# instadeepai/FrameDiPT

Hardware: AMD Instinct MI355X
Metric: residue*diffusion-steps/sec (higher is better)
Workload: dtype fp16

## Files before the change

### framedipt_amd/csrc/edge_transition4.hip

```cpp
#include <type_traits>

#include "common.hpp"
#include "kernels.hpp"

#define E4_CZ 128
#define E4_H 384
#define E4_WAVES 8
#define E4_THREADS (64 * E4_WAVES)
#define E4_BUF 32768
#define E4_WBI (2048 + 64)
#define E4_L1_FR (12 * 8)
#define E4_L2_FR (12 * 24)
#define E4_LF_FR (24 * 4)
#define E4_DZ_FR0 496
#define E4_STREAM_FR 512
#define E4_STREAM_BYTES (E4_STREAM_FR * 1024)
static_assert(E4_L1_FR + E4_L2_FR + E4_LF_FR == 480, "480 weight fragments, then one unused chunk and the down_z chunk");
#define E4X_LF_FR (24 * 8)
#define E4X_DZ_FR0 624
#define E4X_STREAM_FR 640
#define E4X_STREAM_BYTES (E4X_STREAM_FR * 1024)
static_assert(E4_L1_FR + E4_L2_FR + E4X_LF_FR == 576 && E4X_DZ_FR0 + 16 == E4X_STREAM_FR, "fp16x stream: 36 weight chunks, down_z in the last");
#define E4_ZOFF (2 * E4_BUF)
#define E4_VOFF (E4_ZOFF + E4_WAVES * 8192)
// ... 326 lines not shown
        float* bo = a.bias_out + fd_bias_frag_off((long)b * a.H + 4 * half, nt, ii, jj);
        const long hstride = (long)nt * nt * 1024;
        const f32x4 bbv = e4_ldsf4(bbo + 16 * half);
#pragma unroll
        for (int r = 0; r < 4; ++r)
          if (4 * half + r < a.H) bo[r * hstride] = X.accb[r] + bbv[r];
      }
    }
    if constexpr (PZ) {
      const int NJ4 = a.N >> 2;
#pragma unroll
      for (int g = 0; g < 4; ++g) {
        const int row = 8 * E.t.rt + 2 * g + half;
        const u32x2 ow = {fd_cvt_pk(X.accd[4 * g], X.accd[4 * g + 1]), fd_cvt_pk(X.accd[4 * g + 2], X.accd[4 * g + 3])};
        if (E.t.valid && row < M)
          *(u32x2*)(a.pz_out + (((long)row * NJ4 + E.t.jt) * 32 + p) * 4) = ow;
      }
    }
  }
}

#define E4_DR 4
#define E4_CHUNK 16384
#define E4_NSLOT 4
#define E4_NCHUNK 32
#define E4_CFR (E4_CHUNK / 1024)
#define E4_DZ_LDS 49152u
#define E4_DPC (E4_CHUNK / (E4_THREADS * 16))
__device__ __forceinline__ void e4_vm_wait(int n) {
  __builtin_amdgcn_sched_barrier(0);
#define E4_VMC(k) case k: __builtin_amdgcn_s_waitcnt(0x0F70 | ((k) & 15) | (((k) >> 4) << 14)); break;
  switch (n) {
    E4_VMC(1) E4_VMC(2) E4_VMC(3) E4_VMC(4) E4_VMC(5) E4_VMC(6) E4_VMC(7) E4_VMC(8) E4_VMC(9) E4_VMC(10) E4_VMC(11) E4_VMC(12)
    E4_VMC(13) E4_VMC(14) E4_VMC(15) E4_VMC(16) E4_VMC(17) E4_VMC(18) E4_VMC(19) E4_VMC(20)
    default: __builtin_amdgcn_s_waitcnt(0x0F70); break;
  }
#undef E4_VMC
  __builtin_amdgcn_sched_barrier(0);
}
#define E4_PT_Z 24
#define E4_PT_FL 26
__device__ __forceinline__ constexpr int e4_vm_younger(int c) {
  return (E4_NSLOT - 3) * E4_DPC + (c > E4_PT_Z && c <= E4_PT_Z + E4_NSLOT - 2 ? 8 : (c > E4_PT_FL && c <= E4_PT_FL + E4_NSLOT - 2 ? 4 : (c <= E4_NSLOT - 3 ? 14 : 0)));
}
__device__ __forceinline__ constexpr unsigned e4_ring_off(int f) { return (unsigned)(((f / E4_CFR) % E4_NSLOT) * E4_CHUNK + (f % E4_CFR) * 1024); }
struct E4Flat {
  const char* stream;
  unsigned lds0, pa;
  int tid, wave;
};
template <int NCH = E4_NCHUNK>
__device__ __forceinline__ void e4_point(const E4Flat& F, int c) {
  e4_vm_wait(e4_vm_younger(c));
  __builtin_amdgcn_s_barrier();
  __builtin_amdgcn_sched_barrier(0);
  const int cn = (c + E4_NSLOT - 1) % NCH;
  e4_dma_chunk<E4_CHUNK>(F.stream + (size_t)cn * E4_CHUNK, F.lds0 + (unsigned)(cn % E4_NSLOT) * E4_CHUNK, F.tid, F.wave);
}
#define E4_STEP(f_, B_, acc_)                                                                                   \
  do {                                                                                                          \
    if ((f_) + E4_DR - 1 < NCH * E4_CFR) r[((f_) + E4_DR - 1) % E4_DR] = fd_frag(F.pa + e4_ring_off((f_) + E4_DR - 1)); \
    acc_ = fd_mfma32(r[(f_) % E4_DR], B_, acc_);                                                                  \
    __builtin_amdgcn_sched_barrier(0);                                                                          \
  } while (0)

template <bool PZ, bool STZ = true, bool LO = false>
__global__ __launch_bounds__(E4_THREADS, 8 / E4_WAVES) void edge_transition4_flat_kernel(ET2Args a, int n_tiles, int n_wt) {
  constexpr int NCH = (LO ? E4X_STREAM_FR : E4_STREAM_FR) / E4_CFR;
  constexpr int LFW = LO ? 8 : 4;
  extern __shared__ __attribute__((aligned(16))) char smem[];
  const unsigned lds0 = (unsigned)(unsigned long)(__attribute__((address_space(3))) char*)smem;
  const unsigned vec = lds0 + E4_VOFF;
  const unsigned wbi = lds0 + E4_VOFF + E4_VEC_BYTES;
  const int wave = __builtin_amdgcn_readfirstlane(threadIdx.x >> 6);
  auto lane_id = [] {
    int l = __builtin_amdgcn_mbcnt_hi(~0u, __builtin_amdgcn_mbcnt_lo(~0u, 0u));
    asm volatile("" : "+v"(l));
    return l;
  };
  const int lane0 = lane_id(), tid0 = wave * 64 + lane0;
  const int N = a.N, NJ4 = N >> 2, M = a.B * N;
  const char* stream = (const char*)a.stream;
  int tile = blockIdx.x;
  if (tile >= n_tiles) return;
  E4_CLK_BEGIN;
#ifdef E4_PROF
  unsigned ph[8] = {0, 0, 0, 0, 0, 0, 0, 0}, tlast = (unsigned)__builtin_amdgcn_s_memtime();
  const unsigned long long span0 = __builtin_amdgcn_s_memrealtime();
#endif
  E4Tile tc = e4_tile_of(tile * E4_WAVES + wave, n_wt, N, NJ4);
  e4_request_z(a, tc, lane0, lds0 + E4_ZOFF + wave * 8192, M);
#pragma unroll
  for (int c = 0; c < E4_NSLOT - 1; ++c) e4_dma_chunk<E4_CHUNK>(stream + c * E4_CHUNK, lds0 + c * E4_CHUNK, tid0, wave);
  if (tid0 < (PZ ? 168 : 160)) {
    const float* src = tid0 < 96 ? a.b2 + 4 * tid0 : (tid0 < 128 ? a.gamma + 4 * (tid0 - 96) : (tid0 < 160 ? a.beta + 4 * (tid0 - 128) : a.bdz + 4 * (tid0 - 160)));
    fd_dma16(src, vec + (tid0 & ~63) * 16);
  }
  if (a.wb_img && tid0 < 128) fd_dma16((const char*)a.wb_img + tid0 * 16, wbi + (tid0 & ~63) * 16);
  if (tid0 < 4) *(__attribute__((address_space(3))) unsigned*)(unsigned long)(wbi + 2048 + tid0 * 4) = 0u;
  auto fold_ptr = [&](const E4Tile& t, int lane) {
    const unsigned fold_b1 = (unsigned)((const char*)a.b1_img - (const char*)a.a1_img);
    const unsigned ob = fold_b1 + (unsigned)((t.b0 * NJ4 + t.jt) * 16) * 512u, oa = (unsigned)(t.rt * 16) * 512u;
    return oa + (unsigned)(lane >> 5) * (ob - oa) + (lane & 31) * 16;
  };
  auto fold_ld = [&](unsigned off) { return fd_frag((const char*)a.a1_img + off); };
  unsigned fold_base = fold_ptr(tc, lane0);
  hx8 FA[12];
#pragma unroll
  for (int k = 0; k < 12; ++k) FA[k] = fold_ld(fold_base + k * 512);
  auto mask_of = [&](const E4Tile& t, int lane) {
    int row = 8 * t.rt + ((lane & 31) >> 2);
    if (row > M - 1) row = M - 1;
    return a.res_mask[row] * a.res_mask[(row / N) * N + 4 * t.jt + (lane & 3)];
  };
  if (tid0 < 8) *(__attribute__((address_space(3))) float*)(unsigned long)(lds0 + E4_BOFF + tid0 * 4) = (a.wb_img && tid0 < a.H) ? a.bb[tid0] : 0.f;
  float em_req = mask_of(tc, lane0);
  E4Epi E;
  E4EpiTmp X;
#define E4_EPI(k, emr) e4_epi<k, PZ, STZ, emr>(E, X, a, lane_id(), vec, wbi, lds0 + E4_SOFF + wave * 2048, M, lds0 + E4_DZ_LDS)
  fd_dma_wait();
  *(__attribute__((address_space(3))) float*)(unsigned long)(lds0 + E4_MOFF + tid0 * 4) = em_req;
  __syncthreads();
  E4_STAMP(0);
#pragma unroll 1
  for (;;) {
    const int lane = lane_id(), tid = wave * 64 + lane;
    const int p = lane & 31, half = lane >> 5;
    const unsigned zst = lds0 + E4_ZOFF + wave * 8192;
    const unsigned zrow = zst + p * 256;
    E4Flat F;
    F.stream = stream; F.lds0 = lds0; F.pa = lds0 + lane * 16; F.tid = tid; F.wave = wave;
    hx8 r[E4_DR];
#pragma unroll
    for (int m = 0; m < E4_DR - 1; ++m) r[m] = fd_frag(F.pa + e4_ring_off(m));
    hx8 H1[24], H2[24];
    {
      const hx8 SEL = e4_sel(lane, tc.ns);
      hx8 Zf[8];
#pragma unroll
      for (int s = 0; s < 8; ++s) Zf[s] = fd_frag(zrow + (((2 * s) ^ (half ^ (p & 15))) << 4));
      __builtin_amdgcn_sched_barrier(0);
#pragma unroll
      for (int T = 0; T < 12; ++T) {
        f32x16 acc;
#pragma unroll
        for (int q = 0; q < 16; ++q) acc[q] = 0.f;
        acc = fd_mfma32(FA[T], SEL, acc);
#pragma unroll
        for (int s = 0; s < 8; ++s) {
          const int f = 8 * T + s;
          if (f % E4_CFR == E4_CFR / 2) e4_point<NCH>(F, f / E4_CFR);
          E4_STEP(f, Zf[s], acc);
        }
        fd_hand_off(acc, H1[2 * T], H1[2 * T + 1]);
        __builtin_amdgcn_sched_barrier(0);
      }
    }
    E4_STAMP(1);
#pragma unroll
    for (int T = 0; T < 12; ++T) {
      f32x16 acc;
#pragma unroll
      for (int g = 0; g < 4; ++g) {
        const f32x4 bv = e4_ldsf4(vec + 4 * (32 * T + 8 * g + 4 * half));
#pragma unroll
        for (int q = 0; q < 4; ++q) acc[4 * g + q] = bv[q];
      }
#pragma unroll
      for (int s = 0; s < 24; ++s) {
        const int f = E4_L1_FR + 24 * T + s;
        if (f % E4_CFR == E4_CFR / 2) e4_point<NCH>(F, f / E4_CFR);
        E4_STEP(f, H1[s], acc);
      }
      fd_hand_off(acc, H2[2 * T], H2[2 * T + 1]);
      __builtin_amdgcn_sched_barrier(0);
      if (T < 4) {
        const int l3 = lane_id();
        const unsigned zrow3 = lds0 + E4_ZOFF + wave * 8192 + (l3 & 31) * 256 + 8 * (l3 >> 5), zsw = l3 & 15;
#pragma unroll
        for (int u = 0; u < 2; ++u) {
          u32x4 zw;
          const u32x2 z0 = *(e4_lds_w64)(unsigned long)(zrow3 + (((4 * T + 2 * u) ^ zsw) << 4));
          const u32x2 z1 = *(e4_lds_w64)(unsigned long)(zrow3 + (((4 * T + 2 * u + 1) ^ zsw) << 4));
          zw[0] = z0[0]; zw[1] = z0[1]; zw[2] = z1[0]; zw[3] = z1[1];
          H2[2 * T + u] = H2[2 * T + u] + __builtin_bit_cast(hx8, zw);
        }
      }
    }
    E4_STAMP(2);
    const int ntile = tile + gridDim.x;
    const bool has_next = ntile < n_tiles;
    const E4Tile tn = e4_tile_of((has_next ? ntile : tile) * E4_WAVES + wave, n_wt, N, NJ4);
#pragma unroll
    for (int t = 0; t < 4; ++t)
#pragma unroll
      for (int q = 0; q < 16; ++q) E.Y[t][q] = 0.f;
    hx8 FL[4];
#pragma unroll
    for (int s = 0; s < 24; ++s)
#pragma unroll
      for (int u = 0; u < LFW; ++u) {
        const int t = u & 3;
        const int f = E4_L1_FR + E4_L2_FR + LFW * s + u;
        if (f % E4_CFR == E4_CFR / 2) {
          e4_point<NCH>(F, f / E4_CFR);
          if (f / E4_CFR == E4_PT_Z) e4_request_z(a, tn, lane_id(), lds0 + E4_ZOFF + wave * 8192, M);
          if (f / E4_CFR == E4_PT_FL) {
            const unsigned fb = fold_ptr(tc, lane_id());
#pragma unroll
            for (int k = 0; k < 4; ++k) FL[k] = fold_ld(fb + (12 + k) * 512);
          }
        }
        E4_STEP(f, H2[s], E.Y[t]);
      }
    static_assert((E4_L1_FR + E4_L2_FR + 24 * LFW) / E4_CFR == NCH - (LO ? 4 : 2), "stream points behind the final layer");
    if constexpr (LO) {
      e4_point<NCH>(F, NCH - 4);
      e4_point<NCH>(F, NCH - 3);
    }
    e4_point<NCH>(F, NCH - 2);
    e4_point<NCH>(F, NCH - 1);
    {
      const hx8 SEL = e4_sel(lane, tc.ns);
#pragma unroll
      for (int t = 0; t < 4; ++t) E.Y[t] = fd_mfma32(FL[t], SEL, E.Y[t]);
    }
    E4_STAMP(3);
    fold_base = fold_ptr(tn, lane);
#pragma unroll
    for (int k = 0; k < 12; ++k) FA[k] = fold_ld(fold_base + k * 512);
    E.t = tc;
    em_req = mask_of(tn, lane);
    X.moff = lds0 + E4_MOFF + tid * 4;
    X.boff = lds0 + E4_BOFF;
    E4_EPI(0, true); E4_EPI(1, true); E4_EPI(2, true); E4_EPI(3, true); E4_EPI(4, true); E4_EPI(5, true); E4_EPI(6, true);
    E4_STAMP(4);
    if (!has_next) break;
    tile = ntile;
    tc = tn;
    e4_vm_wait(14);
    *(__attribute__((address_space(3))) float*)(unsigned long)(lds0 + E4_MOFF + tid * 4) = em_req;
    E4_STAMP(5);
  }
  fd_dma_wait();
  E4_CLK_END;
#ifdef E4_PROF
  if (tid0 == 0 && blockIdx.x < 256)
    for (int k = 0; k < 8; ++k) e4_prof[blockIdx.x * 8 + k] = ph[k];
  if (tid0 == 0 && blockIdx.x < 1024) {
    e4_span[blockIdx.x * 3] = span0;
    e4_span[blockIdx.x * 3 + 1] = __builtin_amdgcn_s_memrealtime();
    e4_span[blockIdx.x * 3 + 2] = 0;
  }
#endif
}

int fd_edge_transition4_supported(int N) { return N >= 8 && N <= 2048 && N % 4 == 0; }

template <bool LO>
static int e4_launch(const ET2Args& a, hipStream_t st) {
  const int n_wt = ((a.B * a.N + 7) / 8) * (a.N / 4);
  const int n_tiles = cdiv(n_wt, E4_WAVES);
  static FdPerDevice attr_dev;
  const int dev_ = fd_device();
  if (!attr_dev.get(dev_)) {
    if (hipFuncSetAttribute((const void*)edge_transition4_flat_kernel<false, true, LO>, hipFuncAttributeMaxDynamicSharedMemorySize, E4_LDS) != hipSuccess ||
        hipFuncSetAttribute((const void*)edge_transition4_flat_kernel<true, true, LO>, hipFuncAttributeMaxDynamicSharedMemorySize, E4_LDS) != hipSuccess ||
        hipFuncSetAttribute((const void*)edge_transition4_flat_kernel<true, false, LO>, hipFuncAttributeMaxDynamicSharedMemorySize, E4_LDS) != hipSuccess)
      return FDIPT_ELAUNCH;
    attr_dev.set(dev_, 1);
  }
  const int n_cu = fd_cu_count();
  const int cus = a.reserve_cus > 0 && a.reserve_cus < n_cu - 8 ? (n_cu - a.reserve_cus) & ~7 : n_cu;
// ... 26 lines not shown
```

### framedipt_amd/csrc/kernels.hpp

```cpp
#pragma once
#include <hip/hip_runtime.h>
#include <stdint.h>

typedef unsigned short half_t;

struct EdgeTransArgs {
  int B, N;
  const void* z_in;
  void* z_out;
  const float* e;
  const void *w1, *w2, *wf;
  const float *b1, *b2, *bf, *gamma, *beta;
  const float* res_mask;
  float* trace;
  unsigned long long* clock = nullptr;
};

struct EdgeEmbedArgs {
  int B, N, n_rel, rel_off, num_bins;
  const float* pi;
  const float* pj;
  const float* rtab;
  const float* dtab;
  const float* edges;
// ... 69 lines not shown
  unsigned short* kpf = nullptr;
  const float* gamma = nullptr;
  const float* res_mask = nullptr;
};
#define FD_KPF_FRAGS 4

__host__ __device__ __forceinline__ long fd_bias_frag_off(long bh, int nt, int i, int j) {
  return ((((bh * nt + (i >> 5)) * nt + (j >> 5)) * 32 + (i & 31)) * 32) + (j & 31);
}

struct ET2Args {
  int B, N;
  const half_t* z_in;
  half_t* z_out;
  const float* e;
  const half_t* e_h16;
  const float* a1;
  const float* af;
  const void* stream;
  const float *b2, *gamma, *beta, *res_mask;
  float* trace;
  const void* wb_img;
  const float* bb;
  float* bias_out;
  int H;
  const void* a1_img;
  const void* b1_img;
  int reserve_cus = 0;
  unsigned long long* clock = nullptr;
  const void* wdz_img = nullptr;
  const void* wdz_img_lo = nullptr;
  const float* bdz = nullptr;
  half_t* pz_out = nullptr;
};
static inline size_t fd_pz_bytes(int B, int N) { return (size_t)B * N * ((N + 3) / 4) * 256; }
int fd_et3_build_stream(const float* w1, const float* w2, const float* wf, void* stream, hipStream_t st);
size_t fd_et3_stream_bytes();
int fd_edge_transition3(const ET2Args& a, hipStream_t st);
int fd_et3_build_bias_image(const float* wb, int H, float scale, void* img, hipStream_t st);
int fd_edge_transition3_supported(int N);
int fd_et4_build_stream(const float* w1, const float* w2, const float* wf, void* stream, hipStream_t st, int lo = 0);
int fd_et4_set_dz(void* stream, const void* img_hi, const void* img_lo, hipStream_t st, int lo = 0);
size_t fd_et4_stream_bytes(int lo = 0);
int fd_et4_build_bias_image(const float* wb, int H, float scale, void* img, hipStream_t st);
size_t fd_et4_a_image_bytes(int B, int N);
size_t fd_et4_b_image_bytes(int B, int N);
int fd_et4_row_images(const float* rows, int B, int N, void* a_img, void* b_img, hipStream_t st);
int fd_edge_transition4(const ET2Args& a, hipStream_t st, int lo = 0);
int fd_edge_transition4_supported(int N);
int fd_ee2_build_images(const float* w2, const float* w3, void* img, hipStream_t st, int lo = 0);
size_t fd_ee2_image_bytes(int lo = 0);
int fd_edge_embed2(const EdgeEmbedArgs& a, const void* img, hipStream_t st, int lo = 0);

struct ProjArgs {
  int B, N, H, C, K, PT, Np;
  const float* A;
  int lda;
  const void* W;
  const void* W_img;
  const void* W_img_lo = nullptr;
  const float* bias;
  float qscale;
  half_t *Qb, *Kb, *Vt;
  half_t* Vt_lo = nullptr;
  float* pts;
  int zero_pads;
// ... 202 lines not shown
```

### framedipt_amd/csrc/model.hip

```cpp
#include <math.h>
#include <string.h>

#include <vector>

#include "common.hpp"
#include "kernels.hpp"

struct LinW { long w, b; int out, in; };
struct LNW { long g, b; int d; };
#define FD_MAX_BLOCKS 8
#define FD_MAX_TL 4
struct TfLayer { LinW inp, outp, l1, l2; LNW n1, n2; };
struct BlockW {
  long head_w;
  LinW q, kv, qp, kvp, lb, dz, out, rbf;
  LNW ipa_ln;
  LinW skip;
  TfLayer tf[FD_MAX_TL];
  LinW post, t1, t2, t3;
  LNW tln;
  LinW bb;
  LinW et_init, et1, et2, etf;
  LNW et_ln;
};
struct Inventory {
  LinW ne0, ne2, ne4; LNW neln;
  LinW ee0, ee2, ee4; LNW eeln;
  BlockW blk[FD_MAX_BLOCKS];
  LinW tor1, tor2, tor3, torf;
  std::vector<long> offsets;
  int d1, node_in, edge_in, d_t, cb, hid, feat_dim, proj_out;
};

static bool half_mode(const FdiptDims* d) {
  return d->precision == FDIPT_PREC_HALF || (FDIPT_PREC_HALF == FDIPT_PREC_F16 && d->precision == FDIPT_PREC_F16X);
}
static int op_precision(const FdiptDims* d) { return half_mode(d) ? FDIPT_PREC_HALF : d->precision; }

static bool dims_ok(const FdiptDims* d) {
  return d && d->num_blocks >= 1 && d->num_blocks <= FD_MAX_BLOCKS && d->tfmr_layers >= 1 && d->tfmr_layers <= FD_MAX_TL &&
         d->c_s > 0 && (d->c_s % 8) == 0 && d->c_z > 0 && (d->c_z % 8) == 0 && d->no_heads > 0 && d->no_heads <= 16 &&
         d->index_embed == 32 && d->num_bins >= 0 && d->num_bins < 64 && (d->c_skip % 8) == 0 &&
         (d->precision == FDIPT_PREC_F32 || half_mode(d)) && (d->kernel_flags & ~FDIPT_KF_ALL) == 0;
}

static void build_inventory(const FdiptDims* d, Inventory& iv) {
  long off = 0;
  iv.offsets.clear();
  auto push = [&](long n) { iv.offsets.push_back(off); long o = off; off += n; return o; };
  auto lin = [&](int out, int in) { LinW l; l.out = out; l.in = in; l.w = push((long)out * in); l.b = push(out); return l; };
  auto ln = [&](int dd) { LNW l; l.d = dd; l.g = push(dd); l.b = push(dd); return l; };
  const int E = d->index_embed;
  iv.d1 = E + 1 + (d->use_aatype ? 21 : 0);
  iv.node_in = iv.d1 + E;
  iv.edge_in = 2 * iv.d1 + E + d->num_bins;
  const int cs = d->c_s, cz = d->c_z, H = d->no_heads, C = d->c_hidden, Pq = d->no_qk_points, Pv = d->no_v_points;
  iv.d_t = cs + d->c_skip;
  iv.cb = cs / 2;
  iv.hid = 2 * iv.cb + cz;
  iv.feat_dim = H * (cz / 4 + C + Pv * 4);
  iv.proj_out = 3 * H * C + 3 * H * Pq + 3 * H * (Pq + Pv);
  iv.ne0 = lin(cs, iv.node_in); iv.ne2 = lin(cs, cs); iv.ne4 = lin(cs, cs); iv.neln = ln(cs);
  iv.ee0 = lin(cz, iv.edge_in); iv.ee2 = lin(cz, cz); iv.ee4 = lin(cz, cz); iv.eeln = ln(cz);
  for (int b = 0; b < d->num_blocks; ++b) {
    BlockW& k = iv.blk[b];
    k.head_w = push(H);
    k.q = lin(H * C, cs); k.kv = lin(2 * H * C, cs); k.qp = lin(H * Pq * 3, cs); k.kvp = lin(H * (Pq + Pv) * 3, cs);
    k.lb = lin(H, cz); k.dz = lin(cz / 4, cz); k.out = lin(cs, iv.feat_dim); k.rbf = lin(1, 20);
    k.ipa_ln = ln(cs);
    k.skip = lin(d->c_skip, cs);
    for (int l = 0; l < d->tfmr_layers; ++l) {
      TfLayer& t = k.tf[l];
      t.inp = lin(3 * iv.d_t, iv.d_t); t.outp = lin(iv.d_t, iv.d_t); t.l1 = lin(iv.d_t, iv.d_t); t.l2 = lin(iv.d_t, iv.d_t);
      t.n1 = ln(iv.d_t); t.n2 = ln(iv.d_t);
    }
    k.post = lin(cs, iv.d_t);
// ... 956 lines not shown
      } else {
        r.w0l = D + db.lo.et_init; r.w1l = D + db.lo.r4w;
        RC(fd_rowblock(FD_RB_ET4_IMAGES, r, st));
      }
    } else if (p.et == ET_ET3) {
      r.w1 = D + db.ch.a1af; r.b1 = (const float*)(D + db.ch.b1f); r.out = F(w.a1); r.ld_out = iv.hid; r.out2 = F(w.af); r.ld_out2 = cz;
      r.split = iv.hid; r.hid_h16 = (unsigned short*)(W + w.e_bf);
      RC(fd_rowblock(FD_RB_ET_ROWS, r, st));
    } else if (p.et == ET_CHAIN) {
      ChainArgs c;
      c.M = R; c.in = node; c.ld_in = cs; c.w[0] = D + db.ch.et_init; c.b[0] = P + k.et_init.b; c.out_h16 = (unsigned short*)(W + w.e_bf);
      c.out = F(w.e); c.ld_out = iv.cb;
      RC(fd_chain(FD_CHAIN_ETINIT, c, st));
    } else if (p.et == ET_GEMM) {
      RC(lin(k.et_init, node, cs, nullptr, 0, nullptr, 0, F(w.e), iv.cb));
      if (p.bf) RC(fd_f32_to_half((long)R * iv.cb, F(w.e), (half_t*)(W + w.e_bf), st));
    }
    float* tr_ptr = a->trace_edge ? a->trace_edge + (size_t)(b + 1) * NN * cz : nullptr;
    if (a->ev_start && a->ev_start[b]) hipEventRecord((hipEvent_t)a->ev_start[b], st);
    if (p.et == ET_ET4 || p.et == ET_ET3) {
      ET2Args t2;
      t2.B = B; t2.N = N; t2.z_in = (const half_t*)(W + w.z); t2.z_out = (half_t*)(W + w.z); t2.e = F(w.e);
      t2.e_h16 = (const half_t*)(W + w.e_bf);
      t2.a1 = F(w.a1); t2.af = F(w.af); t2.stream = D + (p.et == ET_ET3 ? db.et3 : p.x ? db.et4x : db.et4); t2.b2 = P + k.et2.b; t2.gamma = P + k.et_ln.g;
      t2.beta = P + k.et_ln.b; t2.res_mask = a->res_mask; t2.trace = tr_ptr;
      const DBlock& next = L.blk[b + 1];
      t2.wb_img = p.et_bias ? D + (p.et == ET_ET4 ? next.wb_img4 : next.wb_img3) : nullptr;
      t2.a1_img = W + w.a1img; t2.b1_img = W + w.b1img;
      t2.bb = (const float*)(D + next.bb); t2.bias_out = F(w.bias); t2.H = d->no_heads; t2.reserve_cus = a->reserve_cus;
      if (p.pz) {
        t2.bdz = P + iv.blk[b + 1].dz.b; t2.pz_out = (half_t*)(W + w.pz);
        if (b + 1 == d->num_blocks - 1 && !tr_ptr) t2.z_out = nullptr;
      }
      t2.clock = a->clock_out;
      if (p.et == ET_ET4) RC(fd_edge_transition4(t2, st, p.x));
      else RC(fd_edge_transition3(t2, st));
    } else {
      EdgeTransArgs ta;
      ta.B = B; ta.N = N; ta.z_in = W + w.z; ta.z_out = W + w.z; ta.e = F(w.e);
      ta.w1 = WM(k.et1); ta.w2 = WM(k.et2); ta.wf = WM(k.etf); ta.b1 = P + k.et1.b; ta.b2 = P + k.et2.b; ta.bf = P + k.etf.b;
      ta.gamma = P + k.et_ln.g; ta.beta = P + k.et_ln.b; ta.res_mask = a->res_mask; ta.trace = tr_ptr; ta.clock = a->clock_out;
      RC(fd_edge_transition(op_precision(d), cz, iv.cb, ta, st));
    }
    if (a->ev_stop && a->ev_stop[b]) hipEventRecord((hipEvent_t)a->ev_stop[b], st);
    return FDIPT_OK;
  }
  int heads_stage(const float* node) const {
    const int cs = d->c_s;
    if (p.torsion == NF_GEMM) {
      RC(lin(iv.tor1, node, cs, nullptr, 0, nullptr, 1, F(w.h_a), cs));
      RC(lin(iv.tor2, F(w.h_a), cs, node, cs, nullptr, 0, F(w.h_b), cs));
    } else {
      const bool r16 = p.torsion == NF_ROWS16;
      RowBlockArgs r;
      r.M = R; r.in = node; r.ld_in = cs; r.w0 = D + (r16 ? L.tor16[0][0] : L.ch_tor1); r.w1 = D + (r16 ? L.tor16[1][0] : L.ch_tor2);
      r.w0l = D + (r16 ? L.tor16[0][1] : L.lo_tor1); r.w1l = D + (r16 ? L.tor16[1][1] : L.lo_tor2);
      r.b0 = P + iv.tor1.b; r.b1 = P + iv.tor2.b; r.residual = node; r.ld_res = cs; r.out = F(w.h_b); r.ld_out = cs;
      if (r16) RC(fd_torsion16(r, st));
      else RC(fd_rowblock(FD_RB_TORSION, r, st));
    }
    if (!p.torf_fused) RC(lin32(iv.torf, F(w.h_b), cs, F(w.psi_un), 8));
    const bool atoms = a->atom37 || a->atom14;
    if (atoms && !a->bb_tables) return FDIPT_EINVAL;
    const bool bb_fold = atoms && p.bb_fold;
    RC(fd_score_tail(B, N, a->rigids_t, F(w.quat), F(w.trans), d->coordinate_scaling, F(w.psi_un), 8, a->gt_psi, a->fixed_mask,
                     a->res_mask, a->so3_sigma, a->t, d->r3_min_b, d->r3_max_b, a->rigids, a->psi, a->rot_score, a->trans_score,
                     a->ca_out, p.torf_fused ? F(w.h_b) : nullptr, cs, cs, P + iv.torf.w, P + iv.torf.b, a->so3_score_table,
// ... 156 lines not shown
```

### include/fdipt.h

```cpp
#ifndef FDIPT_H
#define FDIPT_H

#include <stddef.h>
#include <stdint.h>

#ifdef __cplusplus
extern "C" {
#endif

#define FDIPT_OK 0
#define FDIPT_EINVAL (-1)
#define FDIPT_ELAUNCH (-2)
#define FDIPT_ESIZE (-3)

#define FDIPT_PREC_F32 0
#define FDIPT_PREC_BF16 1
#define FDIPT_PREC_F16 2
#define FDIPT_PREC_F16X 3

#define FDIPT_KF_ET3 1
#define FDIPT_KF_GENERIC_PAIR 2
#define FDIPT_KF_GENERIC_ATTN 4
#define FDIPT_KF_UNFUSED_NODE 8
#define FDIPT_KF_UNFOLDED 16
#define FDIPT_KF_NO_MERGE 64
#define FDIPT_KF_ROWS32 128
#define FDIPT_KF_PASS_Z 256
#define FDIPT_KF_POINTS_LAUNCH 512
#define FDIPT_KF_STREAM_ATTN 1024
#define FDIPT_KF_ALL 2015

typedef void* fdipt_stream_t;

typedef struct FdiptDims {
  int32_t c_s;
  int32_t c_z;
  int32_t c_hidden;
  int32_t c_skip;
  int32_t no_heads;
  int32_t no_qk_points;
  int32_t no_v_points;
  int32_t tfmr_heads;
  int32_t tfmr_layers;
  int32_t num_blocks;
  int32_t index_embed;
  int32_t num_bins;
  int32_t use_aatype;
  int32_t precision;
  int32_t kernel_flags;
  float min_bin;
  float max_bin;
  float coordinate_scaling;
  float r3_min_b;
  float r3_max_b;
} FdiptDims;

int fdipt_param_count(const FdiptDims* dims);
int64_t fdipt_param_offset(const FdiptDims* dims, int index);

size_t fdipt_derived_bytes(const FdiptDims* dims);
int fdipt_model_prepare(const FdiptDims* dims, const float* params_f32, void* derived, fdipt_stream_t stream);

size_t fdipt_setup_bytes(const FdiptDims* dims, int B, int N, int n_rel);
// ... 360 lines not shown
```

Measured before the change: 1.212 million.

## Overlap edge-transition epilogue with next tile's layer 1 via finer weight ring

For the PZ fp16 path, the weight stream ring changes from 4×16KB slots to 6×8KB slots, and down_z is preloaded once into LDS. The previous tile's epilogue (z staging and stores, bias MFMA, down_z MFMA, bias and pz stores) is broken into scheduled steps and interleaved with the next tile's layer-1 MFMAs. Fold operands are loaded lazily into a 4-entry rotating buffer to free registers. The goal is to hide epilogue latency and stores behind compute. The cost is much more complex vmcnt bookkeeping, a dump buffer for masked stores, and a new flag that restores the end-of-tile epilogue.

```diff
diff --git a/framedipt_amd/csrc/edge_transition4.hip b/framedipt_amd/csrc/edge_transition4.hip
--- a/framedipt_amd/csrc/edge_transition4.hip
+++ b/framedipt_amd/csrc/edge_transition4.hip
@@ -382,7 +382,8 @@
 #define E4_VMC(k) case k: __builtin_amdgcn_s_waitcnt(0x0F70 | ((k) & 15) | (((k) >> 4) << 14)); break;
   switch (n) {
     E4_VMC(1) E4_VMC(2) E4_VMC(3) E4_VMC(4) E4_VMC(5) E4_VMC(6) E4_VMC(7) E4_VMC(8) E4_VMC(9) E4_VMC(10) E4_VMC(11) E4_VMC(12)
-    E4_VMC(13) E4_VMC(14) E4_VMC(15) E4_VMC(16) E4_VMC(17) E4_VMC(18) E4_VMC(19) E4_VMC(20)
+    E4_VMC(13) E4_VMC(14) E4_VMC(15) E4_VMC(16) E4_VMC(17) E4_VMC(18) E4_VMC(19) E4_VMC(20) E4_VMC(21) E4_VMC(22) E4_VMC(23) E4_VMC(24)
+    E4_VMC(25) E4_VMC(26) E4_VMC(27) E4_VMC(28) E4_VMC(29) E4_VMC(30) E4_VMC(31)
     default: __builtin_amdgcn_s_waitcnt(0x0F70); break;
   }
 #undef E4_VMC
@@ -393,32 +394,227 @@
 __device__ __forceinline__ constexpr int e4_vm_younger(int c) {
   return (E4_NSLOT - 3) * E4_DPC + (c > E4_PT_Z && c <= E4_PT_Z + E4_NSLOT - 2 ? 8 : (c > E4_PT_FL && c <= E4_PT_FL + E4_NSLOT - 2 ? 4 : (c <= E4_NSLOT - 3 ? 14 : 0)));
 }
-__device__ __forceinline__ constexpr unsigned e4_ring_off(int f) { return (unsigned)(((f / E4_CFR) % E4_NSLOT) * E4_CHUNK + (f % E4_CFR) * 1024); }
+template <bool FINE>
+struct E4Ring {
+  static constexpr int CHUNK = FINE ? 8192 : E4_CHUNK, NSLOT = FINE ? 6 : E4_NSLOT, CFR = CHUNK / 1024, DPC = CHUNK / (E4_THREADS * 16);
+  static constexpr int PT_Z = FINE ? 49 : E4_PT_Z, PT_FL = FINE ? 53 : E4_PT_FL;
+  static constexpr int NCH_W = (E4_L1_FR + E4_L2_FR + E4_LF_FR) / CFR;
+  __device__ static constexpr unsigned off(int f) { return (unsigned)(((f / CFR) % NSLOT) * CHUNK + (f % CFR) * 1024); }
+};
+static_assert(E4Ring<true>::NCH_W % E4Ring<true>::NSLOT == 0 && E4Ring<true>::NSLOT * E4Ring<true>::CHUNK == (int)E4_DZ_LDS, "the fine ring turns in whole rounds, below down_z");
 struct E4Flat {
   const char* stream;
   unsigned lds0, pa;
   int tid, wave;
 };
-template <int NCH = E4_NCHUNK>
-__device__ __forceinline__ void e4_point(const E4Flat& F, int c) {
-  e4_vm_wait(e4_vm_younger(c));
+template <bool FINE, int NCH>
+__device__ __forceinline__ void e4_point(const E4Flat& F, int c, int younger) {
+  using R = E4Ring<FINE>;
+  e4_vm_wait(younger);
   __builtin_amdgcn_s_barrier();
   __builtin_amdgcn_sched_barrier(0);
-  const int cn = (c + E4_NSLOT - 1) % NCH;
-  e4_dma_chunk<E4_CHUNK>(F.stream + (size_t)cn * E4_CHUNK, F.lds0 + (unsigned)(cn % E4_NSLOT) * E4_CHUNK, F.tid, F.wave);
+  const int cn = (c + R::NSLOT - 1) % NCH;
+  e4_dma_chunk<R::CHUNK>(F.stream + (size_t)cn * R::CHUNK, F.lds0 + (unsigned)(cn % R::NSLOT) * R::CHUNK, F.tid, F.wave);
 }
 #define E4_STEP(f_, B_, acc_)                                                                                   \
   do {                                                                                                          \
-    if ((f_) + E4_DR - 1 < NCH * E4_CFR) r[((f_) + E4_DR - 1) % E4_DR] = fd_frag(F.pa + e4_ring_off((f_) + E4_DR - 1)); \
+    if ((f_) + E4_DR - 1 < NCH * R::CFR) r[((f_) + E4_DR - 1) % E4_DR] = fd_frag(F.pa + R::off((f_) + E4_DR - 1)); \
     acc_ = fd_mfma32(r[(f_) % E4_DR], B_, acc_);                                                                  \
     __builtin_amdgcn_sched_barrier(0);                                                                          \
   } while (0)
 
+#define E4_EM_T 13
+#define E4_EM_LAT 2
+static_assert(E4_EM_T >= 13 && (E4_EM_LAT == 2 || E4_EM_LAT == 3), "a feature tile's read-backs come before the next one's staging writes");
+#define E4_EM_BL 73
+#define E4_EM_BIAS (E4_EM_BL + 2)
+#define E4_EM_PZ (E4_EM_BIAS + 4)
+#define E4_EM_END (E4_EM_PZ + 13)
+static_assert(E4_EM_BL >= 3 * E4_EM_T + 15, "behind the last feature tile's steps");
+__device__ __attribute__((aligned(16))) unsigned e4_dump[64];
+struct E4Emit {
+  hx8* zB;
+  f32x16 accb, accd;
+  hx8 wf, df[2];
+  u16x8 rb[2];
+  f32x4 bbv;
+  E4Tile t;
+  unsigned long dump;
+};
+__host__ __device__ constexpr int e4_em_stores(int e, bool stz) {
+  int n = 0;
+  for (int t = 0; t < 4; ++t) n += stz && (e - E4_EM_T * t == 13 || e - E4_EM_T * t == 14) ? 1 : 0;
+  return n + (e == E4_EM_BIAS ? 4 : 0) + (e >= E4_EM_PZ && e < E4_EM_END && (e - E4_EM_PZ) % 4 == 0 ? 1 : 0);
+}
+static_assert(1 + E4_EM_END <= 108, "the table ends inside layer 1");
+__host__ __device__ constexpr int e4_l1_vm(int slot, int mode, bool stz) {
+  return mode >= 0 ? (slot % 9 == 1 && slot / 9 + 3 < 12 ? 1 : 0) + e4_em_stores(slot - 1 - mode, stz) : 0;
+}
+__host__ __device__ constexpr int e4f_younger_tail(int c) {
+  using R = E4Ring<true>;
+  return (R::NSLOT - 3) * R::DPC + (c > R::PT_Z && c <= R::PT_Z + R::NSLOT - 2 ? 8 : 0) + (c > R::PT_FL && c <= R::PT_FL + R::NSLOT - 2 ? 4 : 0);
+}
+__host__ __device__ constexpr int e4f_younger(int c, int mode, bool stz) {
+  using R = E4Ring<true>;
+  int n = (R::NSLOT - 3) * R::DPC + (c <= R::NSLOT - 3 ? (mode >= 0 ? 5 : 14) : 0);
+  const int lo = c >= R::NSLOT - 2 ? 9 * (c - (R::NSLOT - 2)) + 5 : 0, hi = 9 * c + 5;
+  for (int s = lo; s < hi; ++s) n += e4_l1_vm(s, mode, stz);
+  return n;
+}
+template <class F, int... I>
+__device__ __forceinline__ void e4_seq(F&& f, std::integer_sequence<int, I...>) { (f(std::integral_constant<int, I>{}), ...); }
+template <int N, class F>
+__device__ __forceinline__ void e4_for(F&& f) { e4_seq(f, std::make_integer_sequence<int, N>{}); }
+static_assert(e4f_younger(3, 0, true) <= 31 && e4f_younger(6, 0, true) <= 31 && e4f_younger(8, 0, true) <= 31 && e4f_younger(3, -1, true) <= 31, "e4_vm_wait's cases");
+
+template <bool TRACE>
+__device__ __forceinline__ void e4_norm(E4Epi& E, hx8* zB, const ET2Args& a, int lane, unsigned vec, unsigned moff, int M) {
+  const int p = lane & 31, half = lane >> 5;
+  E.em = *(const __attribute__((address_space(3))) float*)(unsigned long)(moff);
+  f32x2 u1 = {0.f, 0.f}, u2 = {0.f, 0.f};
+#pragma unroll
+  for (int t = 0; t < 4; ++t)
+#pragma unroll
+    for (int r = 0; r < 16; r += 2) {
+      const f32x2 y = {E.Y[t][r], E.Y[t][r + 1]};
+      u1 += y;
+      u2 = __builtin_elementwise_fma(y, y, u2);
+    }
+  const float s1 = e4_both_halves(u1[0] + u1[1], lane), s2 = e4_both_halves(u2[0] + u2[1], lane);
+  const float mu = s1 * (1.0f / E4_CZ);
+  const float var = fmaxf(s2 * (1.0f / E4_CZ) - mu * mu, 0.f);
+  const float rstd = 1.0f / sqrtf(var + 1e-5f);
+  const f32x2 sa = {rstd, rstd}, sc = {-mu * rstd, -mu * rstd};
+  const int row = 8 * E.t.rt + (p >> 2);
+  const bool valid = E.t.valid && row < M;
+  const long prow = (long)(row < M ? row : M - 1) * a.N + 4 * E.t.jt + (p & 3);
+#pragma unroll
+  for (int t = 0; t < 4; ++t) {
+    const unsigned gml = vec + 4 * (E4_H + 4 * half + 32 * t);
+    const unsigned btl = gml + 4 * E4_CZ;
+#pragma unroll
+    for (int h2 = 0; h2 < 2; ++h2) {
+      f32x4 gm[2], bt[2];
+#pragma unroll
+      for (int k = 0; k < 2; ++k) {
+        gm[k] = e4_ldsf4(gml + 32 * (2 * h2 + k));
+        bt[k] = e4_ldsf4(btl + 32 * (2 * h2 + k));
+      }
+      f32x2 o[4];
+#pragma unroll
+      for (int k = 0; k < 2; ++k) {
+        const int g = 2 * h2 + k;
+        f32x2 o0 = {E.Y[t][4 * g], E.Y[t][4 * g + 1]}, o1 = {E.Y[t][4 * g + 2], E.Y[t][4 * g + 3]};
+        o0 = __builtin_elementwise_fma(o0, sa, sc);
+        o1 = __builtin_elementwise_fma(o1, sa, sc);
+        o[2 * k] = __builtin_elementwise_fma(o0, f32x2{gm[k][0], gm[k][1]}, f32x2{bt[k][0], bt[k][1]});
+        o[2 * k + 1] = __builtin_elementwise_fma(o1, f32x2{gm[k][2], gm[k][3]}, f32x2{bt[k][2], bt[k][3]});
+      }
+#pragma unroll
+      for (int k = 0; k < 4; ++k) o[k] *= f32x2{E.em, E.em};
+      u32x4 zw;
+#pragma unroll
+      for (int k = 0; k < 4; ++k) zw[k] = fd_cvt_pk(o[k][0], o[k][1]);
+      zB[2 * t + h2] = __builtin_bit_cast(hx8, zw);
+      if (TRACE && a.trace && valid) {
+        float* tr_row = a.trace + prow * E4_CZ + 4 * half + 32 * t + 16 * h2;
+#pragma unroll
+        for (int k = 0; k < 2; ++k) *(f32x4*)(tr_row + 8 * k) = f32x4{o[2 * k][0], o[2 * k][1], o[2 * k + 1][0], o[2 * k + 1][1]};
+      }
+    }
+  }
+}
+
+typedef __attribute__((address_space(1))) u16x8 e4_g_u16x8;
+typedef __attribute__((address_space(1))) u32x2 e4_g_u32x2;
+typedef __attribute__((address_space(1))) float e4_g_f32;
+struct E4EmitAddr {
+  unsigned stgw;
+  unsigned wl, ws;
+  unsigned dzl;
+  unsigned rbk;
+  half_t* zd[2];
+};
+template <bool STZ>
+__device__ __forceinline__ E4EmitAddr e4_emit_addr(const E4Tile& t, const ET2Args& a, int lane, unsigned wbi, unsigned stg, int M, unsigned dzf, unsigned long dump) {
+  const int p = lane & 31, half = lane >> 5;
+  E4EmitAddr A;
+  A.stgw = stg + p * 64 + (((p >> 2) & 3) << 4) + 8 * half;
+  A.wl = p < 8 ? wbi + half * 128 + p * 16 : wbi + 2048;
+  A.ws = p < 8 ? 256u : 0u;
+  A.dzl = dzf + lane * 16;
+  A.rbk = stg + (lane >> 2) * 64 + (((lane & 3) ^ ((lane >> 4) & 3)) << 4);
+#pragma unroll
+  for (int k = 0; k < 2; ++k) {
+    const int pr = 16 * k + (lane >> 2), r2 = 8 * t.rt + (pr >> 2);
+    A.zd[k] = nullptr;
+    if constexpr (STZ) {
+      A.zd[k] = a.z_out + ((long)(r2 < M ? r2 : M - 1) * a.N + 4 * t.jt + (pr & 3)) * E4_CZ + 8 * (lane & 3);
+      if (!(t.valid && r2 < M)) A.zd[k] = (half_t*)dump + 8 * (lane & 3);
+    }
+  }
+  return A;
+}
+template <bool STZ, int t, int rel>
+__device__ __forceinline__ void e4_emit_tile(E4Emit& Q, const E4EmitAddr& A) {
+  if constexpr (rel < 4) {
+    if constexpr (STZ) {
+      constexpr int h2 = rel >> 1, k = rel & 1, g = 2 * h2 + k;
+      const u32x4 zw = __builtin_bit_cast(u32x4, Q.zB[2 * t + h2]);
+      *(e4_lds_w64)(unsigned long)(A.stgw ^ (unsigned)(g << 4)) = u32x2{zw[2 * k], zw[2 * k + 1]};
+    }
+  }
+  if constexpr (rel == 4 + E4_EM_LAT || rel == 7 + E4_EM_LAT) Q.accb = fd_mfma32(Q.wf, Q.zB[2 * t + (rel == 7 + E4_EM_LAT)], Q.accb);
+  if constexpr (rel == 5 + E4_EM_LAT || rel == 8 + E4_EM_LAT) Q.accd = fd_mfma32(Q.zB[2 * t + (rel == 8 + E4_EM_LAT)], Q.df[0], Q.accd);
+  if constexpr (rel == 6 + E4_EM_LAT || rel == 9 + E4_EM_LAT) Q.accd = fd_mfma32(Q.zB[2 * t + (rel == 9 + E4_EM_LAT)], Q.df[1], Q.accd);
+  if constexpr (rel == 4 || rel == 7) Q.wf = fd_frag(A.wl + (2 * t + (rel == 7)) * A.ws);
+  if constexpr (rel == 5 || rel == 8) Q.df[0] = fd_frag(A.dzl + (2 * t + (rel == 8)) * 1024);
+  if constexpr (rel == 6 || rel == 9) Q.df[1] = fd_frag(A.dzl + 8192 + (2 * t + (rel == 9)) * 1024);
+  if constexpr (STZ && (rel == 11 || rel == 12)) Q.rb[rel - 11] = *(fd_lds_u16x8)(unsigned long)(A.rbk + 1024 * (rel - 11));
+  if constexpr (STZ && (rel == 13 || rel == 14)) *(e4_g_u16x8*)(A.zd[rel - 13] + 32 * t) = Q.rb[rel - 13];
+}
+template <bool STZ, int e>
+__device__ __forceinline__ void e4_emit(E4Emit& Q, const E4EmitAddr& A, const ET2Args& a, int lane, unsigned vec, int M, unsigned boff) {
+  const int p = lane & 31, half = lane >> 5;
+  if constexpr (e == -1) {
+    const float bd = *(const __attribute__((address_space(3))) float*)(unsigned long)(vec + 4 * (E4_H + 2 * E4_CZ + p));
+#pragma unroll
+    for (int r = 0; r < 16; ++r) {
+      Q.accb[r] = 0.f;
+      Q.accd[r] = bd;
+    }
+  }
+  if constexpr (e >= 0 && e / E4_EM_T < 4) e4_emit_tile<STZ, e / E4_EM_T, e % E4_EM_T>(Q, A);
+  if constexpr (e >= E4_EM_T && e / E4_EM_T <= 4 && e % E4_EM_T + E4_EM_T <= 14) e4_emit_tile<STZ, e / E4_EM_T - 1, e % E4_EM_T + E4_EM_T>(Q, A);
+  if constexpr (e == E4_EM_BL) Q.bbv = e4_ldsf4(boff + 16 * half);
+  if constexpr (e == E4_EM_BIAS) {
+    const int row = 8 * Q.t.rt + (p >> 2), jj = 4 * Q.t.jt + (p & 3), rc = row < M ? row : M - 1;
+    const int b = Q.t.b0 + ((p >> 2) >= Q.t.ns ? 1 : 0), ii = rc - b * a.N, nt = (a.N + 31) >> 5;
+    float* bo = a.bias_out + fd_bias_frag_off((long)b * a.H + 4 * half, nt, ii, jj);
+    const long hstride = (long)nt * nt * 1024;
+    const bool ok = Q.t.valid && row < M;
+#pragma unroll
+    for (int r = 0; r < 4; ++r) {
+      float* dst = ok && 4 * half + r < a.H ? bo + r * hstride : (float*)Q.dump;
+      *(e4_g_f32*)dst = Q.accb[r] + Q.bbv[r];
+    }
+  }
+  if constexpr (e >= E4_EM_PZ && e < E4_EM_END && (e - E4_EM_PZ) % 4 == 0) {
+    constexpr int g = (e - E4_EM_PZ) / 4;
+    const int row = 8 * Q.t.rt + 2 * g + half, NJ4 = a.N >> 2;
+    const u32x2 ow = {fd_cvt_pk(Q.accd[4 * g], Q.accd[4 * g + 1]), fd_cvt_pk(Q.accd[4 * g + 2], Q.accd[4 * g + 3])};
+    half_t* dst = a.pz_out + (((long)(row < M ? row : M - 1) * NJ4 + Q.t.jt) * 32 + p) * 4;
+    *(e4_g_u32x2*)(Q.t.valid && row < M ? dst : (half_t*)Q.dump) = ow;
+  }
+}
+
 template <bool PZ, bool STZ = true, bool LO = false>
 __global__ __launch_bounds__(E4_THREADS, 8 / E4_WAVES) void edge_transition4_flat_kernel(ET2Args a, int n_tiles, int n_wt) {
-  constexpr int NCH = (LO ? E4X_STREAM_FR : E4_STREAM_FR) / E4_CFR;
+  constexpr bool FINE = PZ && !LO;
+  using R = E4Ring<FINE>;
+  constexpr int NCH = FINE ? R::NCH_W : (LO ? E4X_STREAM_FR : E4_STREAM_FR) / R::CFR;
   constexpr int LFW = LO ? 8 : 4;
-  extern __shared__ __attribute__((aligned(16))) char smem[];
+    extern __shared__ __attribute__((aligned(16))) char smem[];
   const unsigned lds0 = (unsigned)(unsigned long)(__attribute__((address_space(3))) char*)smem;
   const unsigned vec = lds0 + E4_VOFF;
   const unsigned wbi = lds0 + E4_VOFF + E4_VEC_BYTES;
@@ -441,7 +637,8 @@
   E4Tile tc = e4_tile_of(tile * E4_WAVES + wave, n_wt, N, NJ4);
   e4_request_z(a, tc, lane0, lds0 + E4_ZOFF + wave * 8192, M);
 #pragma unroll
-  for (int c = 0; c < E4_NSLOT - 1; ++c) e4_dma_chunk<E4_CHUNK>(stream + c * E4_CHUNK, lds0 + c * E4_CHUNK, tid0, wave);
+  for (int c = 0; c < R::NSLOT - 1; ++c) e4_dma_chunk<R::CHUNK>(stream + c * R::CHUNK, lds0 + c * R::CHUNK, tid0, wave);
+  if constexpr (FINE) e4_dma_chunk<16384>(stream + (size_t)E4_DZ_FR0 * 1024, lds0 + E4_DZ_LDS, tid0, wave);
   if (tid0 < (PZ ? 168 : 160)) {
     const float* src = tid0 < 96 ? a.b2 + 4 * tid0 : (tid0 < 128 ? a.gamma + 4 * (tid0 - 96) : (tid0 < 160 ? a.beta + 4 * (tid0 - 128) : a.bdz + 4 * (tid0 - 160)));
     fd_dma16(src, vec + (tid0 & ~63) * 16);
@@ -467,7 +664,14 @@
   float em_req = mask_of(tc, lane0);
   E4Epi E;
   E4EpiTmp X;
+  E4Emit Q;
+  Q.zB = FA + 4;
+  Q.dump = (unsigned long)e4_dump;
+  asm volatile("" : "+s"(Q.dump));
+  bool pend = false;
 #define E4_EPI(k, emr) e4_epi<k, PZ, STZ, emr>(E, X, a, lane_id(), vec, wbi, lds0 + E4_SOFF + wave * 2048, M, lds0 + E4_DZ_LDS)
+#define E4_EMIT(e) e4_emit<STZ, e>(Q, A, a, lane_id(), vec, M, lds0 + E4_BOFF)
+#define E4_EMIT_ADDR e4_emit_addr<STZ>(Q.t, a, lane_id(), wbi, lds0 + E4_SOFF + wave * 2048, M, lds0 + E4_DZ_LDS, Q.dump)
   fd_dma_wait();
   *(__attribute__((address_space(3))) float*)(unsigned long)(lds0 + E4_MOFF + tid0 * 4) = em_req;
   __syncthreads();
@@ -482,30 +686,52 @@
     F.stream = stream; F.lds0 = lds0; F.pa = lds0 + lane * 16; F.tid = tid; F.wave = wave;
     hx8 r[E4_DR];
 #pragma unroll
-    for (int m = 0; m < E4_DR - 1; ++m) r[m] = fd_frag(F.pa + e4_ring_off(m));
+    for (int m = 0; m < E4_DR - 1; ++m) r[m] = fd_frag(F.pa + R::off(m));
     hx8 H1[24], H2[24];
-    {
+    auto layer1 = [&](auto mode_c) __attribute__((always_inline)) {
+      constexpr int MODE = decltype(mode_c)::value;
+      E4EmitAddr A;
+      if constexpr (FINE && MODE >= 0) A = E4_EMIT_ADDR;
       const hx8 SEL = e4_sel(lane, tc.ns);
       hx8 Zf[8];
 #pragma unroll
       for (int s = 0; s < 8; ++s) Zf[s] = fd_frag(zrow + (((2 * s) ^ (half ^ (p & 15))) << 4));
       __builtin_amdgcn_sched_barrier(0);
-#pragma unroll
-      for (int T = 0; T < 12; ++T) {
+      e4_for<12>([&](auto T_c) __attribute__((always_inline)) {
+        constexpr int T = decltype(T_c)::value;
         f32x16 acc;
 #pragma unroll
         for (int q = 0; q < 16; ++q) acc[q] = 0.f;
-        acc = fd_mfma32(FA[T], SEL, acc);
-#pragma unroll
-        for (int s = 0; s < 8; ++s) {
-          const int f = 8 * T + s;
-          if (f % E4_CFR == E4_CFR / 2) e4_point<NCH>(F, f / E4_CFR);
+        acc = fd_mfma32(FA[FINE && MODE >= 0 ? T % 4 : T], SEL, acc);
+        if constexpr (FINE && MODE >= 0) {
+          __builtin_amdgcn_sched_barrier(0);
+          constexpr int e = 9 * T - 1 - MODE;
+          if constexpr (e >= -1 && e < E4_EM_END) E4_EMIT(e);
+          __builtin_amdgcn_sched_barrier(0);
+        }
+        e4_for<8>([&](auto s_c) __attribute__((always_inline)) {
+          constexpr int s = decltype(s_c)::value, f = 8 * T + s;
+          if constexpr (f % R::CFR == R::CFR / 2) {
+            constexpr int young = FINE ? e4f_younger(f / R::CFR, MODE, STZ) : e4_vm_younger(f / R::CFR);
+            e4_point<FINE, NCH>(F, f / R::CFR, young);
+          }
           E4_STEP(f, Zf[s], acc);
-        }
+          if constexpr (FINE) {
+            constexpr int e = 9 * T + s - MODE;
+            if constexpr (MODE >= 0 && e >= -1 && e < E4_EM_END) E4_EMIT(e);
+            if constexpr (MODE >= 0 && s == 0 && T + 3 < 12) FA[(T + 3) % 4] = fold_ld(fold_base + (T + 3) * 512);
+            __builtin_amdgcn_sched_barrier(0);
+          }
+        });
         fd_hand_off(acc, H1[2 * T], H1[2 * T + 1]);
         __builtin_amdgcn_sched_barrier(0);
-      }
-    }
+      });
+    };
+    if constexpr (FINE) {
+      if (!pend) layer1(std::integral_constant<int, -1>{});
+      else layer1(std::integral_constant<int, 0>{});
+    } else
+      layer1(std::integral_constant<int, -1>{});
     E4_STAMP(1);
 #pragma unroll
     for (int T = 0; T < 12; ++T) {
@@ -519,7 +745,7 @@
 #pragma unroll
       for (int s = 0; s < 24; ++s) {
         const int f = E4_L1_FR + 24 * T + s;
-        if (f % E4_CFR == E4_CFR / 2) e4_point<NCH>(F, f / E4_CFR);
+        if (f % R::CFR == R::CFR / 2) e4_point<FINE, NCH>(F, f / R::CFR, FINE ? e4f_younger_tail(f / R::CFR) : e4_vm_younger(f / R::CFR));
         E4_STEP(f, H1[s], acc);
       }
       fd_hand_off(acc, H2[2 * T], H2[2 * T + 1]);
@@ -552,10 +778,10 @@
       for (int u = 0; u < LFW; ++u) {
         const int t = u & 3;
         const int f = E4_L1_FR + E4_L2_FR + LFW * s + u;
-        if (f % E4_CFR == E4_CFR / 2) {
-          e4_point<NCH>(F, f / E4_CFR);
-          if (f / E4_CFR == E4_PT_Z) e4_request_z(a, tn, lane_id(), lds0 + E4_ZOFF + wave * 8192, M);
-          if (f / E4_CFR == E4_PT_FL) {
+        if (f % R::CFR == R::CFR / 2) {
+          e4_point<FINE, NCH>(F, f / R::CFR, FINE ? e4f_younger_tail(f / R::CFR) : e4_vm_younger(f / R::CFR));
+          if (f / R::CFR == R::PT_Z) e4_request_z(a, tn, lane_id(), lds0 + E4_ZOFF + wave * 8192, M);
+          if (f / R::CFR == R::PT_FL) {
             const unsigned fb = fold_ptr(tc, lane_id());
 #pragma unroll
             for (int k = 0; k < 4; ++k) FL[k] = fold_ld(fb + (12 + k) * 512);
@@ -563,13 +789,15 @@
         }
         E4_STEP(f, H2[s], E.Y[t]);
       }
-    static_assert((E4_L1_FR + E4_L2_FR + 24 * LFW) / E4_CFR == NCH - (LO ? 4 : 2), "stream points behind the final layer");
+    static_assert((E4_L1_FR + E4_L2_FR + 24 * LFW) / R::CFR == NCH - (FINE ? 0 : LO ? 4 : 2), "stream points behind the final layer");
     if constexpr (LO) {
-      e4_point<NCH>(F, NCH - 4);
-      e4_point<NCH>(F, NCH - 3);
-    }
-    e4_point<NCH>(F, NCH - 2);
-    e4_point<NCH>(F, NCH - 1);
+      e4_point<FINE, NCH>(F, NCH - 4, e4_vm_younger(NCH - 4));
+      e4_point<FINE, NCH>(F, NCH - 3, e4_vm_younger(NCH - 3));
+    }
+    if constexpr (!FINE) {
+      e4_point<FINE, NCH>(F, NCH - 2, e4_vm_younger(NCH - 2));
+      e4_point<FINE, NCH>(F, NCH - 1, e4_vm_younger(NCH - 1));
+    }
     {
       const hx8 SEL = e4_sel(lane, tc.ns);
 #pragma unroll
@@ -577,18 +805,32 @@
     }
     E4_STAMP(3);
     fold_base = fold_ptr(tn, lane);
-#pragma unroll
-    for (int k = 0; k < 12; ++k) FA[k] = fold_ld(fold_base + k * 512);
+    if constexpr (FINE) pend = has_next && !a.epi_end;
+#pragma unroll
+    for (int k = 0; k < (FINE ? 3 : 12); ++k) FA[k] = fold_ld(fold_base + k * 512);
+    if (FINE && !pend) FA[3] = fold_ld(fold_base + 3 * 512);
     E.t = tc;
     em_req = mask_of(tn, lane);
     X.moff = lds0 + E4_MOFF + tid * 4;
     X.boff = lds0 + E4_BOFF;
-    E4_EPI(0, true); E4_EPI(1, true); E4_EPI(2, true); E4_EPI(3, true); E4_EPI(4, true); E4_EPI(5, true); E4_EPI(6, true);
+    if constexpr (FINE) {
+      e4_norm<STZ>(E, Q.zB, a, lane_id(), vec, X.moff, M);
+      Q.t = tc;
+      if (!pend) {
+        const E4EmitAddr A = E4_EMIT_ADDR;
+        e4_for<E4_EM_END + 1>([&](auto e_c) __attribute__((always_inline)) { E4_EMIT(decltype(e_c)::value - 1); });
+#pragma unroll
+        for (int k = 4; k < 12; ++k) FA[k] = fold_ld(fold_base + k * 512);
+      }
+    } else {
+      E4_EPI(0, true); E4_EPI(1, true); E4_EPI(2, true); E4_EPI(3, true); E4_EPI(4, true); E4_EPI(5, true); E4_EPI(6, true);
+    }
     E4_STAMP(4);
     if (!has_next) break;
     tile = ntile;
     tc = tn;
-    e4_vm_wait(14);
+    if (FINE && pend) e4_vm_wait(5);
+    else e4_vm_wait(14);
     *(__attribute__((address_space(3))) float*)(unsigned long)(lds0 + E4_MOFF + tid * 4) = em_req;
     E4_STAMP(5);
   }
diff --git a/framedipt_amd/csrc/kernels.hpp b/framedipt_amd/csrc/kernels.hpp
--- a/framedipt_amd/csrc/kernels.hpp
+++ b/framedipt_amd/csrc/kernels.hpp
@@ -125,6 +125,7 @@
   const void* wdz_img_lo = nullptr;
   const float* bdz = nullptr;
   half_t* pz_out = nullptr;
+  int epi_end = 0;
 };
 static inline size_t fd_pz_bytes(int B, int N) { return (size_t)B * N * ((N + 3) / 4) * 256; }
 int fd_et3_build_stream(const float* w1, const float* w2, const float* wf, void* stream, hipStream_t st);
diff --git a/framedipt_amd/csrc/model.hip b/framedipt_amd/csrc/model.hip
--- a/framedipt_amd/csrc/model.hip
+++ b/framedipt_amd/csrc/model.hip
@@ -41,7 +41,7 @@
   return d && d->num_blocks >= 1 && d->num_blocks <= FD_MAX_BLOCKS && d->tfmr_layers >= 1 && d->tfmr_layers <= FD_MAX_TL &&
          d->c_s > 0 && (d->c_s % 8) == 0 && d->c_z > 0 && (d->c_z % 8) == 0 && d->no_heads > 0 && d->no_heads <= 16 &&
          d->index_embed == 32 && d->num_bins >= 0 && d->num_bins < 64 && (d->c_skip % 8) == 0 &&
-         (d->precision == FDIPT_PREC_F32 || half_mode(d)) && (d->kernel_flags & ~FDIPT_KF_ALL) == 0;
+         (d->precision == FDIPT_PREC_F32 || half_mode(d)) && (d->kernel_flags & ~(FDIPT_KF_ALL | FDIPT_KX_ET4_EPI_END)) == 0;
 }
 
 static void build_inventory(const FdiptDims* d, Inventory& iv) {
@@ -1064,7 +1064,7 @@
         t2.bdz = P + iv.blk[b + 1].dz.b; t2.pz_out = (half_t*)(W + w.pz);
         if (b + 1 == d->num_blocks - 1 && !tr_ptr) t2.z_out = nullptr;
       }
-      t2.clock = a->clock_out;
+      t2.clock = a->clock_out; t2.epi_end = (d->kernel_flags & FDIPT_KX_ET4_EPI_END) != 0;
       if (p.et == ET_ET4) RC(fd_edge_transition4(t2, st, p.x));
       else RC(fd_edge_transition3(t2, st));
     } else {
diff --git a/include/fdipt.h b/include/fdipt.h
--- a/include/fdipt.h
+++ b/include/fdipt.h
@@ -29,6 +29,7 @@
 #define FDIPT_KF_POINTS_LAUNCH 512
 #define FDIPT_KF_STREAM_ATTN 1024
 #define FDIPT_KF_ALL 2015
+#define FDIPT_KX_ET4_EPI_END 4096
 
 typedef void* fdipt_stream_t;
 
```

After: 1.223 million (median of 6 runs). No clear change (+0.9%).
